# rampasek/DrVAE

Hardware: AMD Instinct MI355X
Metric: DrVAE ELBO training samples/sec (batch x L) (higher is better)
Workload: dtype f32; 1 GPU; cfg2: DrVAE bortezomib shape: 978 genes, z1=z3=100, enc-z1 800, dec-x 600, enc-z3/dec-z1 200, batch 150/GPU, L=2; global_batch=150, L=2, parallelism=dp1, launch=hipGraph replay, feed=resident, side_chain_cus=64, rccl_ranks=0, params=2321758

## Files before the change

### drvae_amd/_lib.py

```python
import ctypes as C
import os

_HERE = os.path.dirname(os.path.abspath(__file__))
LIB_PATH = os.path.join(_HERE, 'libdrvae_hip.so')

ACT = {'identity': 0, 'elu': 1, 'softplus': 2, 'sigmoid': 3, 'tanh': 4, 'relu': 5, 'leaky_relu': 6, 'selu': 7,
       'softsign': 8, 'cos': 9}
GAUSS_LOGVAR, GAUSS_SIGMA = 0, 1
REC_KIND = {'binary': 0, 'poisson': 1}
EPI_PLAIN, EPI_FWD, EPI_BWD, EPI_KLQ = 0, 1, 2, 3

_f, _i32, _i64, _u64, _p = C.c_float, C.c_int32, C.c_int64, C.c_uint64, C.c_void_p


class GemmDesc(C.Structure):
    _fields_ = [('M', _i32), ('N', _i32), ('K', _i32), ('a_kcontig', _i32), ('b_kcontig', _i32),
                ('A', _p), ('lda', _i64), ('A2', _p), ('lda2', _i64), ('K1', _i32), ('a_kscale', _p),
                ('B', _p), ('ldb', _i64), ('C', _p), ('ldc', _i64), ('alpha', _f), ('beta', _f),
                ('epilogue', _i32), ('scale', _p), ('bias', _p), ('split', _i32), ('act0', _i32), ('act1', _i32),
                ('shift0', _f), ('shift1', _f), ('resid', _p), ('ldr', _i64), ('resid_cols', _i32),
                ('yref', _p), ('ldy', _i64), ('a_colsum', _p), ('colsum_beta', _f), ('flags', _i32),
                ('pub_flag', _p), ('pub_ctr', _p), ('pub_add', _i32), ('tune', _p)]


class GemmTune(C.Structure):
    _fields_ = [('tiling', _i32), ('opt', _i32 * 10)]


class Wait(C.Structure):
    _fields_ = [('flag', _p), ('ctr', _p), ('add', _i32), ('max_spins', _i32), ('err', _p)]


class PriorKl(C.Structure):
    _fields_ = [('coef', _p), ('raw', _p), ('kl_min', _f), ('mu', _p), ('ld', _i64)]


class AdamHyper(C.Structure):
    _fields_ = [('lr', _f), ('beta1', _f), ('beta2', _f), ('eps', _f), ('weight_decay', _f), ('gscale', _f)]


class ClipRecord(C.Structure):
    _fields_ = [('norm', _f), ('coef', _f), ('skip', _i32), ('n_skipped', _i32)]


class ClipState(C.Structure):
    _fields_ = [('step', _i32), ('reserved', _i32), ('max_norm', C.c_double), ('rec', ClipRecord)]


SUMSQ_PER_BLOCK, SUMSQ_MAX_BLOCKS = 8192, 1024


class Publish(C.Structure):
    _fields_ = [('flag', _p), ('ctr', _p), ('add', _i32)]
# ... 226 lines not shown
```

### drvae_amd/csrc/optim.hip

```cpp
#include "dv_common.h"
#include <cstring>

namespace {

struct AdamC {
    float lr_over_bc1, inv_unused, bc2_sqrt, eps, wd, one_minus_b1, b2, one_minus_b2, gscale;
};

__device__ __forceinline__ void adam_consts(float lr, float b1, float b2, const int32_t* step_dev, float* step_size,
                                            float* bc2_sqrt, int n_skipped = 0) {
    const double t = (double)(step_dev[0] - n_skipped);
    const double bc1 = 1.0 - pow((double)b1, t);
    const double bc2 = 1.0 - pow((double)b2, t);
    *step_size = (float)((double)lr / bc1);
    *bc2_sqrt = (float)sqrt(bc2);
}

__device__ __forceinline__ void adam_one(float& p, float g, float& m, float& v, float step_size, float bc2_sqrt,
                                         float eps, float wd, float w1, float b2, float w2, float gscale) {
#pragma clang fp contract(off)
    g = g * gscale;
    if (wd != 0.f) g = __builtin_fmaf(wd, p, g);
    m = __builtin_fmaf(w1, g - m, m);
    v = __builtin_fmaf(w2 * g, g, v * b2);
// ... 5 lines not shown
    int bad = 0;
    for (int i = 0; i < n_halt; ++i)
        bad |= __hip_atomic_load(halt + 2 * i, __ATOMIC_RELAXED, __HIP_MEMORY_SCOPE_AGENT) != 0;
    return bad;
}

struct AdamGate {
    int32_t* flag;
    const int32_t* ctr;
    int add;
    int32_t* err;
    int max_spins;
    int64_t lo, hi;
};

template <bool CLIP>
__global__ __launch_bounds__(256) void adam_kernel(float* __restrict__ p, const float* __restrict__ g,
                                                   float* __restrict__ m, float* __restrict__ v, int64_t n, float lr,
                                                   float b1, float b2, float eps, float wd, float gscale_in,
                                                   const int32_t* __restrict__ step_dev, int vec4, AdamGate gate,
                                                   const int32_t* __restrict__ halt, int n_halt,
                                                   const dv_clip_record* __restrict__ clip) {
    __shared__ float sc[2];
    __shared__ int halted;
    bool need = false;
    if (gate.flag != nullptr) {
        const int64_t per = vec4 ? 4 : 1, span = (int64_t)blockDim.x * per;
        const int64_t bstride = (int64_t)gridDim.x * span;
        need = gate.hi > (vec4 ? ((n >> 2) << 2) : n) && gate.lo < n;
        for (int64_t e0 = blockIdx.x * span; e0 < n; e0 += bstride) need = need || (e0 < gate.hi && e0 + span > gate.lo);
    }
    if (threadIdx.x == 0) {
        int want = 0, seen = 0;
        if (need) {
            want = gate.ctr[0] + gate.add;
            seen = __hip_atomic_load(gate.flag, __ATOMIC_ACQUIRE, __HIP_MEMORY_SCOPE_AGENT);
        }
        int h = any_halt(halt, n_halt);
        if (CLIP) {
            if (clip->skip) h = 1;
            else adam_consts(lr, b1, b2, step_dev, &sc[0], &sc[1], clip->n_skipped);
        } else {
            adam_consts(lr, b1, b2, step_dev, &sc[0], &sc[1]);
        }
        if (need && seen - want < 0) {
// ... 8 lines not shown
            }
            atomicAdd(gate.err + 1, (int32_t)(wall_clock64() - t0));
            h = h || any_halt(halt, n_halt);
        }
        halted = h;
    }
    if (need) {
        __syncthreads();
        __builtin_amdgcn_fence(__ATOMIC_ACQUIRE, "agent");
    }
    __syncthreads();
    if (halted) return;
    const float step_size = sc[0], bc2_sqrt = sc[1];
    const float gscale = CLIP ? gscale_in * clip->coef : gscale_in;
    const float w1 = (float)(1.0 - (double)b1), w2 = (float)(1.0 - (double)b2);
    const int64_t stride = (int64_t)gridDim.x * blockDim.x;
    const int64_t t0 = blockIdx.x * (int64_t)blockDim.x + threadIdx.x;
    if (vec4) {
        const int64_t n4 = n >> 2;
        float4* p4 = reinterpret_cast<float4*>(p);
        const float4* g4 = reinterpret_cast<const float4*>(g);
        float4* m4 = reinterpret_cast<float4*>(m);
        float4* v4 = reinterpret_cast<float4*>(v);
        for (int64_t i = t0; i < n4; i += stride) {
            float4 pp = p4[i], gg = g4[i], mm = m4[i], vv = v4[i];
            adam_one(pp.x, gg.x, mm.x, vv.x, step_size, bc2_sqrt, eps, wd, w1, b2, w2, gscale);
            adam_one(pp.y, gg.y, mm.y, vv.y, step_size, bc2_sqrt, eps, wd, w1, b2, w2, gscale);
            adam_one(pp.z, gg.z, mm.z, vv.z, step_size, bc2_sqrt, eps, wd, w1, b2, w2, gscale);
            adam_one(pp.w, gg.w, mm.w, vv.w, step_size, bc2_sqrt, eps, wd, w1, b2, w2, gscale);
            p4[i] = pp;
            m4[i] = mm;
            v4[i] = vv;
// ... 361 lines not shown
    return c ? c + 1 : dv_src_tag;
}

extern "C" const char* dv_error_string(int code) {
    switch (code) {
        case DV_OK: return "ok";
        case DV_ERR_ARG: return "invalid argument";
        case DV_ERR_LAUNCH: return "kernel launch failed";
        case DV_ERR_UNSUPPORTED: return "unsupported configuration";
        default: return "unknown error";
    }
}

static int adam_launch(float* p, const float* g, float* m, float* v, int64_t n, float lr, float beta1, float beta2,
                       float eps, float weight_decay, float gscale, const int32_t* step_dev, const AdamGate& gate,
                       const int32_t* halt, int32_t n_halt, dv_stream_t stream, const dv_clip_record* clip = nullptr) {
    DV_REQUIRE(n >= 0 && n_halt >= 0 && (halt || n_halt == 0));
    if (n == 0) return DV_OK;
    DV_REQUIRE(p && g && m && v && step_dev);
    auto al = [](const void* q) { return (reinterpret_cast<uintptr_t>(q) & 15) == 0; };
    const int vec4 = al(p) && al(g) && al(m) && al(v);
    int64_t blocks = ((vec4 ? (n >> 2) : n) + 255) / 256;
    if (blocks < 1) blocks = 1;
    if (vec4 && gate.flag == nullptr && n >= (int64_t(16) << 20)) {
        const dim3 grid((unsigned)(blocks > 16384 ? 16384 : blocks));
        if (clip)
            hipLaunchKernelGGL(adam_stream_kernel<true>, grid, dim3(256), 0, ST(stream), p, g, m, v, n, lr, beta1, beta2, eps,
                               weight_decay, gscale, step_dev, halt, n_halt, clip);
        else
            hipLaunchKernelGGL(adam_stream_kernel<false>, grid, dim3(256), 0, ST(stream), p, g, m, v, n, lr, beta1, beta2, eps,
                               weight_decay, gscale, step_dev, halt, n_halt, clip);
        DV_RETURN_LAUNCH();
    }
    if (blocks > 2048) blocks = 2048;
    if (clip)
        hipLaunchKernelGGL(adam_kernel<true>, dim3((unsigned)blocks), dim3(256), 0, ST(stream), p, g, m, v, n, lr, beta1,
                           beta2, eps, weight_decay, gscale, step_dev, vec4, gate, halt, n_halt, clip);
    else
        hipLaunchKernelGGL(adam_kernel<false>, dim3((unsigned)blocks), dim3(256), 0, ST(stream), p, g, m, v, n, lr, beta1,
                           beta2, eps, weight_decay, gscale, step_dev, vec4, gate, halt, n_halt, clip);
    DV_RETURN_LAUNCH();
}

extern "C" int dv_adam_l2_gated(float* p, const float* g, float* m, float* v, int64_t n, const dv_adam_hyper* h,
                                const int32_t* step_dev, const dv_wait* gate, int64_t lo, int64_t hi,
                                const int32_t* halt, int32_t n_halt, dv_stream_t stream) {
    DV_REQUIRE(h != nullptr && gate != nullptr);
    DV_REQUIRE(gate->flag && gate->ctr && gate->err && gate->max_spins > 0 && lo >= 0 && hi >= lo && hi <= n);
    return adam_launch(p, g, m, v, n, h->lr, h->beta1, h->beta2, h->eps, h->weight_decay, h->gscale, step_dev,
                       AdamGate{gate->flag, gate->ctr, gate->add, gate->err, gate->max_spins, lo, hi}, halt, n_halt, stream);
}

static int adamax_launch(float* p, const float* g, float* m, float* u, int64_t n, const dv_adam_hyper* h,
                         const int32_t* step_dev, const int32_t* halt, int32_t n_halt, dv_stream_t stream,
                         const dv_clip_record* clip) {
    DV_REQUIRE(h != nullptr && n >= 0 && n_halt >= 0 && (halt || n_halt == 0));
    if (n == 0) return DV_OK;
    DV_REQUIRE(p && g && m && u && step_dev);
    int64_t blocks = (n + 255) / 256;
    if (blocks > 4096) blocks = 4096;
    if (clip)
        hipLaunchKernelGGL(adamax_kernel<true>, dim3((unsigned)blocks), dim3(256), 0, ST(stream), p, g, m, u, n, h->lr,
                           h->beta1, h->beta2, h->eps, h->weight_decay, h->gscale, step_dev, halt, n_halt, clip);
// ... 134 lines not shown
```

### drvae_amd/data.py

```python
import types

import numpy as np
import torch

from . import kernels as K


class DrVAEDataset(torch.utils.data.Dataset):

    FIELDS = ('x1', 'x2', 's', 'y', 'has_x2', 'has_y')

    def __init__(self, x1, x2, s, y, has_x2, has_y):
        n = x1.size(0)
        assert x2.size(0) == n and x1.size(1) == x2.size(1)
        assert y.size(0) == n and s.size(0) == n and has_x2.size(0) == n and has_y.size(0) == n
        self.x1, self.x2, self.s, self.y, self.has_x2, self.has_y = x1, x2, s, y, has_x2, has_y

    def __getitem__(self, index):
        return tuple(getattr(self, f)[index] for f in self.FIELDS)

    def __len__(self):
        return self.x1.size(0)

    def to(self, device):
# ... 415 lines not shown
                self._pending = self._reference_epoch()
            idx, self._pending = self._pending[0], self._pending[1:]
            return idx.to(self.ds.x1.device)
        if self.mode == 'sampler':
            return torch.multinomial(self.weights, self.global_batch, replacement=True, generator=self.gen)
        R = self.world
        parts = [m[torch.multinomial(w, c * R, replacement=True, generator=self.gen)].reshape(R, c)
                 for m, w, c in zip(self.members, self.gweights, self.group_counts) if c > 0]
        return torch.cat(parts, 1).reshape(-1)

    def feed(self, idx=None):
        if self.mode == 'sampler' and self.bucketed:
            self.engine.set_structure_universal(self.batch_size, n_tot=self._n_tot(), carry_s=self._carry)
        p = self.engine.plan
        p.feed_active = False
        idx = self.next_indices() if idx is None else idx
        if self.dp is not None and idx.numel() == self.global_batch:
            if self.mode == 'sampler':
                zero = torch.zeros((), dtype=torch.int32, device=idx.device)
                p.gcounts_dev.copy_(torch.stack([self.hx32[idx].sum() if self.engine.cfg.has_pert else zero,
                                                 self.hy32[idx].sum() if self.engine.cfg.has_y else zero]))
            idx = idx.reshape(self.world, self.batch_size)[self.rank]
        self._idx32.copy_(idx)
        K.rows_gather(p.XSRC[:p.B], self.ds.x1, self._idx32)
        if self.engine.cfg.has_pert:
            K.rows_gather(p.XSRC[p.B:], self.ds.x2, self._idx32)
        if self.engine.cfg.use_s:
            p.set_s_device(self.ds.s.reshape(-1)[idx])
        if self.mode == 'sampler':
            if self.engine.cfg.has_pert:
# ... 11 lines not shown
```

### drvae_amd/engine.py

```python
import math
import os
from collections import OrderedDict
from dataclasses import dataclass, field
from typing import List, Optional, Tuple

import numpy as np
import torch

from . import kernels as K
from . import tuning as T
from ._lib import GAUSS_LOGVAR, GAUSS_SIGMA
from .arena import N_LOSS, ParamArena, span
from .chain import X3_PARTS, _Chain, _Lin, _pad4
from .plan import LOSS_IDX, _Plan
from .schedule import DUAL, EVAL, EVALUATE, FORK_JOIN, LOSS, TRAIN, StepSchedule, StepSync, _Branch, heads_route


MATMUL_CHOICES = ('fp32',) + tuple(X3_PARTS)
assert MATMUL_CHOICES == ('fp32', 'bf16x3', 'bf16x2', 'bf16x1')


@dataclass
class StepConfig:
    kind: str = 'drvae'
# ... 294 lines not shown
            assert s is not None, 'use_s: the nuisance classes of the batch are needed'
            p = self._set_batch(x1, x2, y, has_x2, has_y, counts)
            if p.carry_s:
                sd = (s if torch.is_tensor(s) else torch.as_tensor(np.asarray(s))).reshape(-1).to(self.dev)
                if len(p.rows) != sd.numel():
                    sd = sd.index_select(0, torch.as_tensor(p.rows, device=self.dev))
                p.set_s_device(sd)
                return p
            sv = np.asarray(s.cpu() if torch.is_tensor(s) else s).astype(np.int64).reshape(-1)
            p.set_s_host(sv[p.rows])
            return p
        return self._set_batch(x1, x2, y, has_x2, has_y, counts)

    def _set_batch(self, x1, x2, y, has_x2, has_y, counts=None):
        cfg = self.cfg
        if self.universal and self.universal_ok():
            hy = np.asarray(has_y.cpu() if torch.is_tensor(has_y) else has_y).reshape(-1)
            p = self.set_structure_universal(len(hy), self.universal_pair_slots, self.universal_labeled_range,
                                             n_tot=None if counts is None else counts[0], carry_s=cfg.use_s)
            p.feed_active = False
            if counts is not None:
                p.gcounts_dev.copy_(torch.tensor([int(counts[1]), int(counts[2])], dtype=torch.int32))
            p.XSRC[:p.B].copy_(x1)
            i32 = lambda a: torch.as_tensor(np.asarray(a.cpu() if torch.is_tensor(a) else a).reshape(-1).astype(np.int32))
            if cfg.has_pert:
                if x2 is None:
                    assert has_x2 is None or not np.asarray(has_x2.cpu() if torch.is_tensor(has_x2) else has_x2).any(), \
                        'has_x2 marks pairs but x2 is None'
                    p.XSRC[p.B:].zero_()
                    p.hx_dev.zero_()
# ... 15 lines not shown
        p.XSRC[:p.B].copy_(x1.index_select(0, sel) if sel is not None else x1)
        if x2 is not None and cfg.has_pert:
            p.XSRC[p.B:].copy_(x2.index_select(0, sel) if sel is not None else x2)
        if cfg.has_y and cfg.cont:
            yv = np.asarray(y.cpu() if torch.is_tensor(y) else y).astype(np.float32).reshape(n_in, -1) \
                if y is not None else np.zeros((n_in, cfg.dim_y), np.float32)
            p.ylab.copy_(torch.from_numpy(np.ascontiguousarray(yv[rows])))
        elif cfg.has_y:
            yv = np.asarray(y.cpu() if torch.is_tensor(y) else y).astype(np.int64).reshape(-1) if y is not None \
                else np.zeros(n_in, np.int64)
            p.set_labels_host(yv[rows])
        return p

    def set_noise(self, noise):
        p, cfg = self.plan, self.cfg
        self._noise_stale = True
        t = lambda a: torch.as_tensor(np.ascontiguousarray(a), dtype=torch.float32)
        rows, L = p.rows, cfg.L
        p.EX[:p.B].copy_(t(np.asarray(noise['nx1'])[rows]))
        if p.Np:
            pr = rows[p.pair_host]
            p.EX[p.B:].copy_(t(np.asarray(noise['nx2'])[pr]))
            p.E2.copy_(t(np.asarray(noise['ez2'])[:, pr].reshape(L * p.Np, -1)))
        p.E1.copy_(t(np.asarray(noise['ez1'])[:, rows].reshape(L * p.B, -1)))
        if cfg.has_pert:
            p.E2F.copy_(t(np.asarray(noise['ez2F'])[:, rows].reshape(L * p.B, -1)))
        if cfg.has_y and p.Mf:
            ez3 = np.asarray(noise['ez3'])
            slot = p.fp_slot_host
            if p.universal:
                hy, yv, i = p.hy_dev.cpu().numpy().astype(bool), p.y_dev.cpu().numpy(), p.fp_i_host
                slot = np.where(hy[i] & (slot == yv[i]), 0, slot)
            p.E3.copy_(t(ez3[p.fp_l_host, slot, rows[p.fp_i_host]]))
        if cfg.has_y and cfg.cont:
            p.EY.copy_(t(np.asarray(noise['ey'])[:, rows].reshape(L * p.B, -1)))

    def draw_noise(self, bump=True):
        n = 1
        if self._rec == 'main' and self._tail.noise_ahead:
            self._rng_pending = n
            return
        lo = 0
        if not (self.training and self.add_noise and self.cfg.add_noise_var > 0):
            lo = self.plan.B + self.plan.Np
        self._fill_noise(self.plan, lo, keeps=self.training)
        self._noise_stale = True
        if bump:
            K.counter_add(self.rng_ctr, n)
        else:
            self._rng_pending = n

    def _fill_noise(self, p, lo=0, keeps=True):
        if p.drop_sites and keeps:
            K.fill_noise_rows(p.noise, p.noise_table[lo:], self.seed, self.rng_ctr)
            p.masks_injected = False
        else:
            K.fill_normal_rows(p.noise, p.noise_desc[lo:p.n_normal_rows], self.seed, self.rng_ctr)

    @property
    def _drop(self):
        return bool(self.training and self.plan.drop_sites)

    def dropout_sites(self):
        return [dict(s) for s in self.plan.drop_sites]

    def set_dropout_masks(self, masks):
        p = self.plan
        index = {(s['chain'], s['layer']): i for i, s in enumerate(p.drop_sites)}
        given = {(index[k] if not isinstance(k, (int, np.integer)) else int(k)): v for k, v in masks.items()}
        assert sorted(given) == list(range(len(p.drop_sites))), 'set_dropout_masks: a mask for every site'
        for i, v in given.items():
            p.drop_sites[i]['mask'].copy_(torch.as_tensor(np.ascontiguousarray(v), dtype=torch.float32))
        p.masks_injected = True
        self._noise_stale = True

    def _route(self):
        return heads_route(self, self.plan, TRAIN if self.fuse_bwd else LOSS if self.training else EVALUATE)

    def beta_pert(self):
        cfg = self.cfg
        if cfg.anneal_perturb_rate_itermax > 0:
            return anneal_coef(self.iters, cfg.anneal_perturb_rate_itermax, cfg.anneal_perturb_rate_offset)
        return 1.

    def forward(self):
        cfg, p = self.cfg, self.plan
        if not self.fuse_bwd and self.dev.type == 'cuda' and not torch.cuda.is_current_stream_capturing():
            self.join_side()
        p.set_beta(self.beta_pert())
# ... 37 lines not shown
                    z2 = None
                else:
                    K.kl_rows_fwd(*zp[0], **zp[1])
            if z2 is not None:
                K.kl_rows_fwd(*z2[0], **z2[1])
            return
        with self.branch:
            self._side_forward(Qmu, Qlv, Z1blk, r)
        if mode == FORK_JOIN:
            return
        self.branch.join()
        if self.fuse_bwd:
            return
        self._loss_scalars()

    def _encoder_forward(self, rec, r):
        cfg, p = self.cfg, self.plan
        B, Np, L, Z1 = p.B, p.Np, cfg.L, cfg.dim_z1
        sigma = cfg.add_noise_var if (self.training and self.add_noise and cfg.add_noise_var > 0) else 0.0
        Z1blk = p.ZDEC[:L * B]
        fd = p.live_feed if (self.fuse_bwd and self.training) else None
        start_park = self.sync.wait('next_step', self.step_dev, add=0) if (rec == 'main' and self._tail.tail_gated) else None
        masks = None
        if p.universal:
            gc = None
            if p.global_counts:
                gc = getattr(fd, 'gcounts', None) if fd is not None else p.gcounts_dev
                assert gc is not None, 'this plan normalises by global counts: the feed carries none (DeviceBatcher.bind(dp=...))'
            masks = dict(n_tot=p.n_tot, gcounts=gc, kl_rate=cfg.kl_qz2pz2_rate, pert_rate=cfg.pertloss_rate,
                         yl_rate=cfg.yloss_rate, beta=p.beta_dev, c_nll=p.c_nll, w_recl=p.w_recl,
                         hx=(fd.hx32 if fd is not None else p.hx_dev) if cfg.has_pert else None,
                         hy=(fd.hy32 if fd is not None else p.hy_dev) if cfg.has_y else None,
                         y=(fd.y32 if fd is not None else p.y_dev) if cfg.has_y else None,
                         c_klz2=p.c_klz2 if cfg.has_pert else None, c_yl=p.c_yl, w_pert=p.w_pert, w_yl=p.w_yl,
# ... 5 lines not shown
            lab = cfg.has_y and not cfg.cont and (not p.universal or p.one_slot is not None)
            K.batch_feed(p.XIN, fd.x1, fd.x2, fd.y32, fd.table, fd.n_batches, self.step_dev, fd.base, park=start_park,
                         pair_rows=p.pair_idx if Np else None, noise=p.EX if sigma else None, sigma=sigma,
                         has_y=p.has_y_i32 if (lab and not p.universal) else None, L=L,
                         label_r=p.label_r if (lab and not p.universal) else None,
                         fp_i=p.fp_q if lab else None, fp_lab=p.fp_lab_i32 if lab else None,
                         fp_slot=p.fp_slot_dev if lab else None, fp_cls=p.fp_cls if (lab and p.Mf) else None,
                         onehot=p.Z3IN[:, cfg.dim_z3:] if (lab and p.Mf) else None, n_classes=cfg.dim_y,
                         onehot2=p.FPIN[:, Z1:] if (lab and p.Mf) else None,
                         yf=fd.yf if (cfg.has_y and cfg.cont) else None,
                         ylab=p.ylab if (cfg.has_y and cfg.cont) else None, masks=masks)
            if cfg.use_s:
                assert p.carry_s and getattr(fd, 's32', None) is not None, 'use_s: this feed does not carry the nuisance classes'
                K.nuisance_feed(p.SOHe, p.SOHd, p.s_cls, fd.s32, table=fd.table, n_batches=fd.n_batches, ctr=self.step_dev,
                                base=fd.base, pair_rows=p.pair_idx if Np else None, L=L)
        else:
            K.rows_gather(p.XIN, p.XSRC, p.xin_idx, noise=p.EX if sigma else None, sigma=sigma, park=start_park)
        if r.sample_epi:
            Q = p.c_enc.forward(p.enc_in, heads=dict(sample=dict(
                eps=p.E12, out=p.ZDEC[:p.o3], n_src=B, seg_ptr=p.zseg_ptr, seg_rows=p.zseg_rows,
                out4=p.FPIN[:, :Z1] if r.fprop_from_heads else None, out4_ptr=p.fp_ptr_ext if r.fprop_from_heads else None)),
                drop=self._drop)
            Qmu, Qlv = Q[:, :Z1], Q[:, Z1:]
        else:
            Q = p.c_enc.forward(p.enc_in, drop=self._drop)
            Qmu, Qlv = Q[:, :Z1], Q[:, Z1:]
            K.reparam_fwd(p.ZDEC[:p.o3], Qmu, Qlv, p.E12, src_idx=p.z_src_idx)
        if cfg.has_pert:
            pub1 = self.sync.pub('z1', self.step_dev) if rec == 'main' else None
            if r.sample_epi:
                p.c_z2F.forward([Z1blk], resid=Z1blk, publish=pub1, heads=dict(sample=dict(
                    eps=p.E2F, out=p.Z2F, n_src=L * B, sub=Z1blk, out2=p.D, out3=p.ZDEC if Np else None,
# ... 435 lines not shown
        if self.clip_rec is not None:
            assert not (t and (t.adam_gated or t.cap_fork or t.side_adam)), 'a clipped sweep has no gated form'
            K.clip_norm(a.grad[:n], self.clip_state, gscale=gscale, adamax=cfg.optim_alg == 'adamax')
            step = K.adamax_l2_clip if cfg.optim_alg == 'adamax' else K.adam_l2_clip
            step(a.param[:n], a.grad[:n], a.exp_avg[:n], a.exp_avg_sq[:n], self.clip_state,
                 lr=cfg.learning_rate, weight_decay=cfg.weight_decay, gscale=gscale, halt=self.sync_err)
            return
        if t and t.adam_gated:
            if cfg.has_y:
                lc, g0 = self.L_clf[0], a.grad.storage_offset()
                lo = min(lc.dW.storage_offset(), lc.db.storage_offset()) - g0
                hi = max(lc.dW.storage_offset() + span(lc.dW), lc.db.storage_offset() + lc.db.numel()) - g0
            else:
                lo, hi = 0, 4
            kw['gate'] = self.sync.gate('clf_dw' if t.tail_gated else 'tail', self.step_dev, lo, hi)
            n = t.hs if t.side_adam else n
        if t and t.cap_fork:
            kw['gate'] = self.sync.gate('tail', self.step_dev, 0, 4)
        step(a.param[:n], a.grad[:n], a.exp_avg[:n], a.exp_avg_sq[:n], self.step_dev, lr=cfg.learning_rate,
             weight_decay=cfg.weight_decay, gscale=gscale, halt=self.sync_err, **kw)

    def clip_stats(self):
        if self.clip_rec is None:
            raise RuntimeError('clip_stats: the engine was built without max_grad_norm')
        self.join_side()
        return K.clip_record_values(self.clip_rec)

    def train_step(self, noise=None, allreduce=None):
        self.training = True
        self.join_side()
# ... 23 lines not shown
```

### drvae_amd/fit.py

```python
import time
import warnings
from collections import OrderedDict

import numpy as np
import torch

from . import engine as E
from . import metrics as MET


class EarlyStopping:

    def __init__(self, epochs, early_stop, patience=50, patience_increase=15, improvement_threshold=0.999,
                 memory_length=3, save_model_after=0):
        self.epochs, self.early_stop = epochs, early_stop
        self.patience, self.patience_increase = patience, patience_increase
        self.improvement_threshold = improvement_threshold
        self.memory_length, self.save_model_after = memory_length, save_model_after
        self.best = -np.inf
        self.rolling = np.array([], dtype=float)
        self.since_improvement = 0
        self.snapshotted = False

    def update(self, epoch, valid_obj):
# ... 736 lines not shown
            K.recon_rows(rows, ll, x, x_rec, x_std, bias=bias[:2] if bias is not None else None,
                         sd_shift=bias[2] if bias is not None else 0.0)
        else:
            K.recon_row_stats(rows, x, x_rec)
            K.nll_rows_fwd(ll, x, x_rec, x_std, mode=GAUSS_SIGMA)
        K.col_moments(None, x, x_rec, sel=sel, part=part, r_bias=bias[0] if bias is not None else None)
        K.recon_finalize(out4, rows, part, X, sel=sel, n=n, ll=ll)

    def run(self):
        m, kind = self.model, self.model.kind
        eng = m.engine()
        eng.join_side()
        eng.iters = m.finished_training_iters
        self.plan.set_beta(eng.beta_pert())
        self.graph.replay()
        eng._noise_stale = True
        if self.dp is not None:
            from . import dist as D
            D.allreduce_sum(self.pack)
            self.graph_final.replay()
        v = dict(zip(self.names, self.vec.cpu().tolist()))
        perf = OrderedDict()
        perf['losses'] = OrderedDict((k, torch.tensor(v['loss_' + k])) for k in self.loss_keys)
        parts = []
        if kind != 'pvae' and self.cont:
            for k in ('rmse', 'r2', 'pearr'):
                perf['y_' + k] = v['y_' + k]
            parts.append('Y: RMSE: {:.3f} R2: {:.3f} Pearson: {:.3f}'.format(perf['y_rmse'], perf['y_r2'], perf['y_pearr']))
        elif kind != 'pvae':
            for k in ('acc', 'auroc', 'aupr'):
                perf['y_' + k] = v['y_' + k]
# ... 16 lines not shown
```

### drvae_amd/kernels.py

```python
import ctypes as C
import math
import os
from typing import Any, NamedTuple, Optional

import torch

from . import _lib
from ._lib import ACT, EPI_BWD, EPI_FWD, EPI_KLQ, EPI_PLAIN, GAUSS_LOGVAR, GAUSS_SIGMA, GemmDesc


def _stream():
    return C.c_void_p(torch.cuda.current_stream().cuda_stream)


def _f32(t, name='tensor', any_device=False):
    if t is None:
        return None
    if not ((t.is_cuda or any_device) and t.dtype == torch.float32):
        raise RuntimeError('drvae_amd kernels need CUDA/HIP float32 tensors (%s is %s on %s); there is no CPU '
                           'fallback' % (name, t.dtype, t.device))
    if t.dim() >= 1 and t.numel() > 0 and t.stride(-1) != 1 and t.size(-1) != 1:
        raise RuntimeError('%s must have unit inner stride' % name)
    return t.data_ptr()

# ... 295 lines not shown
class Publish(NamedTuple):
    flag: Any
    ctr: Any
    add: int = 1


class Gate(NamedTuple):
    flag: Any
    ctr: Any
    add: int
    err: Any
    lo: int
    hi: int


def _wait(park):
    if park is None:
        return None
    park = Wait(*park)
    w = _lib.Wait()
    w.flag, w.ctr, w.err, w.add = _i32(park.flag), _i32(park.ctr), _i32(park.err), park.add
    w.max_spins = WAIT_SPINS if park.max_spins is None else park.max_spins
    return C.byref(w)


def _publish(pub):
    if pub is None:
        return None
    pub = Publish(*pub)
    w = _lib.Publish()
# ... 590 lines not shown
        arr[i].row_len = term[4] if len(term) > 4 else 1
    if after is None and not bump:
        _lib.check(_lib.load().dv_loss_assemble(arr, len(terms), _f32(w_elbo), _f32(w_cmpl), _f32(loss), hp, hn,
                                                _f32(accum), _stream()), 'dv_loss_assemble')
    else:
        _lib.check(_lib.load().dv_loss_assemble_after(_wait(after), arr, len(terms), _f32(w_elbo), _f32(w_cmpl), _f32(loss),
                                                      _bump(bump), hp, hn, _f32(accum), _stream()), 'dv_loss_assemble_after')


def axpby(y, x, a=1.0, b=0.0):
    assert x.is_contiguous() and y.is_contiguous() and x.numel() == y.numel()
    _lib.check(_lib.load().dv_axpby(_f32(x), a, _f32(y), b, x.numel(), _stream()), 'dv_axpby')


def adam_l2(p, g, m, v, step_dev, *, lr, beta1=0.9, beta2=0.999, eps=1e-8, weight_decay=0.0, gscale=1.0, gate=None,
            halt=None):
    assert p.is_contiguous() and g.is_contiguous() and m.is_contiguous() and v.is_contiguous()
    hp, hn = _halt(halt)
    h = _lib.AdamHyper(lr=lr, beta1=beta1, beta2=beta2, eps=eps, weight_decay=weight_decay, gscale=gscale)
    if gate is None:
        _lib.check(_lib.load().dv_adam_l2(_f32(p), _f32(g), _f32(m), _f32(v), p.numel(), C.byref(h), _i32(step_dev), hp, hn,
                                          _stream()), 'dv_adam_l2')
    else:
        gate = Gate(*gate)
        _lib.check(_lib.load().dv_adam_l2_gated(_f32(p), _f32(g), _f32(m), _f32(v), p.numel(), C.byref(h), _i32(step_dev),
                                                _wait(Wait(gate.flag, gate.ctr, gate.err, gate.add)), gate.lo, gate.hi, hp, hn,
                                                _stream()), 'dv_adam_l2_gated')


def adamax_l2(p, g, m, u, step_dev, *, lr, beta1=0.9, beta2=0.999, eps=1e-8, weight_decay=0.0, gscale=1.0, halt=None):
    assert p.is_contiguous() and g.is_contiguous() and m.is_contiguous() and u.is_contiguous()
    hp, hn = _halt(halt)
    h = _lib.AdamHyper(lr=lr, beta1=beta1, beta2=beta2, eps=eps, weight_decay=weight_decay, gscale=gscale)
    _lib.check(_lib.load().dv_adamax_l2(_f32(p), _f32(g), _f32(m), _f32(u), p.numel(), C.byref(h), _i32(step_dev), hp, hn,
                                        _stream()), 'dv_adamax_l2')


CLIP_STATE_WORDS = C.sizeof(_lib.ClipState) // 4
_CLIP_STEP, _CLIP_MAX_NORM, _CLIP_REC = (getattr(_lib.ClipState, f).offset // 4 for f in ('step', 'max_norm', 'rec'))
assert _CLIP_STEP == 0 and CLIP_STATE_WORDS % 2 == 0 and _CLIP_MAX_NORM % 2 == 0


def sumsq_partials(n):
    per, cap = _lib.SUMSQ_PER_BLOCK, _lib.SUMSQ_MAX_BLOCKS
# ... 107 lines not shown
```

### drvae_amd/schedule.py

```python
import contextlib
import ctypes
import gc
import os
import weakref
from typing import NamedTuple

import torch

from . import kernels as K
from . import tuning as T


def _masked_stream(bits, device):
    hip = ctypes.CDLL('libamdhip64.so')
    st = ctypes.c_void_p()
    arr = (ctypes.c_uint32 * len(bits))(*bits)
    with torch.cuda.device(device):
        rc = hip.hipExtStreamCreateWithCUMask(ctypes.byref(st), len(bits), arr)
    if rc != 0:
        raise RuntimeError('hipExtStreamCreateWithCUMask failed: %d' % rc)
    import atexit

    def _destroy(handle=st.value):
        try:
# ... 56 lines not shown

class Tail(NamedTuple):
    dual: bool = False
    late: bool = False
    adam_gated: bool = False
    side_adam: bool = False
    hs: int = 0
    side_loss: bool = False
    cap_fork: bool = False
    tail_gated: bool = False
    noise_ahead: bool = False
    klz2_on_main: bool = False
    fold_join: bool = False
    late_fork: bool = False
    fold_rows: bool = False


TRAIN, LOSS, EVALUATE = 'train pass', 'loss pass, separate backward', 'evaluation pass'
NLL_ROUTES = {'heads': 'NLLP', 'rec': 'NLL', 'raw_cs_eval': 'NLLC', 'raw_eval': 'NLL', 'raw_cs': 'NLLC', 'fwdbwd': 'NLL',
              'fwd': 'NLL'}


class HeadsRoute(NamedTuple):
    sample_epi: bool
    fprop_from_heads: bool
    z3_in_heads: bool
    fprop_tail: bool
    nll: str
    rows: str
    raw_last: bool
# ... 55 lines not shown
            self._forked = False
            self._ctx = torch.cuda.stream(self.side)
            self._ctx.__enter__()
        return self

    def __exit__(self, *exc):
        if self.on:
            self._ctx.__exit__(*exc)

    def join(self):
        if self.on:
            torch.cuda.current_stream().wait_stream(self.side)


_CAPTURE_STATE = ('_graphs', '_side_graph', 'noise_ahead', '_graph_key', '_graph_feed', '_graph_mmd_sig',
                  '_captured_allreduce', '_graph_noise')


class StepSchedule:

    def _init_schedule_state(self):
        self._graphs = []
        self._side_graph = None
        self.noise_ahead = False
        self._graph_key = None
        self._graph_feed = None
        self._graph_mmd_sig = None
        self._captured_allreduce = None
        self._graph_noise = None
        self._captures = {}
        self._rec = 'both'
        self._tail = Tail()
        self._after_decoder_bwd = None
        self._rng_pending = 0
        self._ctr_bumped = False
        self._noise_stale = True
        self._flag_side = None
        self._flags_ok = None
        self._side_cus = None
        self._since_poll = 0
        self._sync_host = None
        self._sync_event = None

    def stash_capture(self):
        assert self._graph_key == self.plan.key, 'stash_capture right after capture(): another plan is current'
        self._captures[self.plan.key] = {k: getattr(self, k) for k in _CAPTURE_STATE}

    def use_capture(self, key):
        cap = self._captures.get(key)
        if cap is None or cap['_graph_feed'] is not self._plans[key].live_feed or \
                cap['_graph_noise'] not in (None, self.add_noise):
            return False
        if self._graph_key != key:
            for k, v in cap.items():
                setattr(self, k, v)
            self.plan = self._plans[key]
            self._noise_stale = True
        return True

    def _mode(self):
        return EVAL if not self.fuse_bwd else DUAL if self._rec != 'both' else FORK_JOIN

    def _step_tail(self, split_kind, on_gpu=None):
        cfg, p = self.cfg, self.plan
        branch_on = self.branch.on if on_gpu is None else bool(self.concurrent and cfg.has_y and on_gpu)
        clip = cfg.max_grad_norm is not None
        if not (self.sched == 5 and self._dual_capable(on_gpu) and self._latency_bound() and
                (self._flags_usable() if on_gpu is None else on_gpu) and (cfg.has_y or not (split_kind or clip))):
            return Tail(late_fork=bool(branch_on and not self._latency_bound()))
        late_ok = bool(not cfg.cont and cfg.optim_alg == 'adam' and (self.clf_small if cfg.has_y else True))
        late = late_ok and (split_kind is True or (split_kind is False and not clip))
        side_ok, hs = self._side_adam_layout()
        side_adam = late and not split_kind and side_ok
        cap_fork = bool(split_kind == 'captured' and side_ok and late_ok and cfg.has_y and T.get('dp_fork') and not clip)
        side_loss = side_adam or (late and split_kind is True and len(self.L_decx) > 1)
        tail_gated = side_adam and (p.live_feed is not None or T.get('tail_gate') == 2)
        klz2_on_main = not cfg.cont and cfg.has_y and not p.every_row_anything
        fold_join = side_loss and cfg.has_pert and (p.B * cfg.dim_z1 + 255) // 256 <= 256 and (p.B + 3) // 4 <= 256
        noise_ahead = bool((late or cap_fork) and not p.drop_sites)
        fold_rows = bool(T.get('fold_rows') and not split_kind and not clip and not p.drop_sites and cfg.kind == 'drvae'
                         and not cfg.cont and self.clf_small and cfg.clf_z1z2 and fold_join and side_loss and noise_ahead
                         and getattr(K.z2f_post_bwd, 'fold_rows', False) and getattr(K.smalln_fwd, 'fold_rows', False))
        return Tail(dual=True, late=late, adam_gated=late and not split_kind, side_adam=side_adam, hs=hs, side_loss=side_loss,
                    cap_fork=cap_fork, tail_gated=tail_gated, noise_ahead=noise_ahead, klz2_on_main=klz2_on_main,
                    fold_join=fold_join, fold_rows=fold_rows)

    @contextlib.contextmanager
    def _recording(self, chain, tail):
        self._rec, self._tail = chain, tail
        try:
            yield
        finally:
            self._rec, self._tail = 'both', Tail()

    def _launch_sequence(self, allreduce=None, draw=True, optimizer=True):
        self.fuse_bwd = True
        try:
            if draw:
                self.draw_noise(bump=False)
            self.forward()
# ... 15 lines not shown
        self.training = True
        self.plan.set_beta(self.beta_pert())
        side = torch.cuda.Stream()
        side.wait_stream(torch.cuda.current_stream())
        with torch.cuda.stream(side):
            self.draw_noise(bump=False)
            self._rng_pending = 0
            self.forward()
            self.backward()
        torch.cuda.current_stream().wait_stream(side)
        torch.cuda.synchronize()
        self._graphs = []
        self._side_graph = None
        tail = self._step_tail(split_for_allreduce)
        self.noise_ahead = tail.noise_ahead
        self._noise_stale = True
        gc.collect()
        gc_was_on = gc.isenabled()
        gc.disable()
        try:
            with self._recording('main' if tail.dual else 'both', tail):
                self._capture_main(split_for_allreduce)
            if tail.dual:
                self.sync_side_counters()
                self.flag_side.wait_stream(torch.cuda.current_stream())
                gs = torch.cuda.CUDAGraph()
                with torch.cuda.graph(gs, stream=self.flag_side), self._recording('side', tail):
                    self._launch_sequence(draw=False, optimizer=False)
                self._side_graph = gs
        finally:
            if gc_was_on:
# ... 82 lines not shown
                for _ in range(4):
                    self.replay()
                e0, e1 = torch.cuda.Event(enable_timing=True), torch.cuda.Event(enable_timing=True)
                e0.record()
                for _ in range(steps):
                    self.replay()
                e1.record()
                e1.synchronize()
                t = e0.elapsed_time(e1)
            if t < best[1]:
                best = (n, t)
        torch.cuda.synchronize()
        for dst, src in zip(state, keep):
            dst.copy_(src)
        self.iters = iters
        self._noise_stale = True
        self.plan.set_beta(self.beta_pert())
        torch.cuda.synchronize()
        self._side_cus = best[0]
        return best[0]

    @property
    def flag_side(self):
        if self._flag_side is None:
            self._flag_side = torch.cuda.Stream(device=self.dev)
        return self._flag_side

    def _probe(self, side):
        probe = torch.zeros(4, dtype=torch.int32, device=self.dev)
        torch.cuda.synchronize()
        K.flag_wait(probe[0:1], probe[1:2], probe[2:4], add=1, max_spins=20000)
# ... 83 lines not shown
            g = torch.cuda.CUDAGraph()
            with torch.cuda.graph(g):
                self._launch_sequence(allreduce=self._captured_allreduce)
            self._graphs = [g]

    def replay(self, allreduce=None):
        assert self._graph_key == self.plan.key, 'batch structure changed: capture again'
        assert self._graph_feed is self.plan.live_feed, 'input source changed (epoch feed <-> explicit batch): capture again'
        assert self._graph_mmd_sig == getattr(self.plan, 'mmd_sig', None), \
            'use_MMD: the nuisance classes of the batch changed (the penalty compares row sets): capture again'
        self.plan.set_beta(self.beta_pert())
        self.plan.masks_injected = False
        if self.noise_ahead and self._noise_stale:
            self._fill_noise(self.plan)
            self._noise_stale = False
        self._graphs[0].replay()
        if self._side_graph is not None:
            with torch.cuda.stream(self.flag_side):
                self._side_graph.replay()
        if len(self._graphs) == 3:
            a = self.arena
            w_early = allreduce.start(a.xchg[a.late_end:])
            self._graphs[1].replay()
            w_late = allreduce.start(a.xchg[:a.late_end])
            allreduce.finish(w_early)
            allreduce.finish(w_late)
            self._graphs[2].replay()
        elif len(self._graphs) == 2:
            if self._side_graph is not None:
                torch.cuda.current_stream().wait_stream(self.flag_side)
# ... 7 lines not shown
```

### drvae_amd/tuning.py

```python
import os

DEFAULTS = {
    'sched': 5,
    'fuse_heads': 1,
    'raw_heads': 1,
    'tail_gate': 1,
    'concurrent': 1,
    'nll_cs': 1,
    'mmd_explicit': 1,
    'fold_rows': 1,
    'dp_fork': 1,
}

CHOICES = {'sched': (3, 5), 'fuse_heads': (0, 1), 'raw_heads': (1, 2), 'tail_gate': (1, 2), 'concurrent': (0, 1),
           'nll_cs': (1, 2), 'mmd_explicit': (0, 1), 'dp_fork': (0, 1), 'fold_rows': (0, 1)}


def _parse():
    out = dict(DEFAULTS)
    for kv in filter(None, os.environ.get('DRVAE_TUNE', '').split(',')):
        k, _, v = kv.partition('=')
        k = k.strip()
        if k not in DEFAULTS:
            raise ValueError('DRVAE_TUNE: unknown switch %r (known: %s)' % (k, ', '.join(sorted(DEFAULTS))))
        out[k] = int(v)
        if out[k] not in CHOICES[k]:
            raise ValueError('DRVAE_TUNE: %s=%d is not a schedule (known: %s)' % (k, out[k], CHOICES[k]))
    return out


# ... 14 lines not shown
```

### include/drvae_hip.h

```cpp
#ifndef DRVAE_HIP_H
#define DRVAE_HIP_H

#include <stdint.h>

#ifdef __cplusplus
extern "C" {
#endif

typedef void* dv_stream_t;

#define DV_ABI_VERSION 12

enum { DV_OK = 0, DV_ERR_ARG = -1, DV_ERR_LAUNCH = -2, DV_ERR_UNSUPPORTED = -3 };

enum {
    DV_ACT_IDENTITY = 0, DV_ACT_ELU = 1, DV_ACT_SOFTPLUS = 2, DV_ACT_SIGMOID = 3, DV_ACT_TANH = 4,
    DV_ACT_RELU = 5, DV_ACT_LEAKY_RELU = 6, DV_ACT_SELU = 7, DV_ACT_SOFTSIGN = 8, DV_ACT_COS = 9
};

enum { DV_GAUSS_LOGVAR = 0, DV_GAUSS_SIGMA = 1 };

enum { DV_EPI_PLAIN = 0, DV_EPI_FWD = 1, DV_EPI_BWD = 2, DV_EPI_KLQ = 3 };

int dv_abi_version(void);
// ... 563 lines not shown
int dv_axpby(const float* x, float a, float* y, float b, int64_t n, dv_stream_t stream);

typedef struct dv_adam_hyper {
    float lr;
    float beta1;
    float beta2;
    float eps;
    float weight_decay;
    float gscale;
} dv_adam_hyper;
int dv_adam_l2(float* p, const float* g, float* m, float* v, int64_t n, const dv_adam_hyper* h,
               const int32_t* step_dev, const int32_t* halt, int32_t n_halt, dv_stream_t stream);
int dv_adam_l2_gated(float* p, const float* g, float* m, float* v, int64_t n, const dv_adam_hyper* h,
                     const int32_t* step_dev, const dv_wait* gate, int64_t lo, int64_t hi, const int32_t* halt,
                     int32_t n_halt, dv_stream_t stream);
int dv_adamax_l2(float* p, const float* g, float* m, float* u, int64_t n, const dv_adam_hyper* h,
                 const int32_t* step_dev, const int32_t* halt, int32_t n_halt, dv_stream_t stream);
typedef struct dv_clip_record {
    float norm;
    float coef;
    int32_t skip;
    int32_t n_skipped;
} dv_clip_record;
typedef struct dv_clip_state {
    int32_t step;
    int32_t reserved;
    double max_norm;
    dv_clip_record rec;
} dv_clip_state;
#define DV_SUMSQ_PER_BLOCK 8192
// ... 18 lines not shown
```

Baseline: 1.659 million samples/s.

## Gather next step's encoder inputs inside the gated Adam kernel as a rider

```diff
diff --git a/drvae_amd/_lib.py b/drvae_amd/_lib.py
--- a/drvae_amd/_lib.py
+++ b/drvae_amd/_lib.py
@@ -37,6 +37,11 @@
 
 class AdamHyper(C.Structure):
     _fields_ = [('lr', _f), ('beta1', _f), ('beta2', _f), ('eps', _f), ('weight_decay', _f), ('gscale', _f)]
+
+
+class AdamRider(C.Structure):
+    _fields_ = [('halt', _p), ('n_halt', _i32), ('n', _i32), ('W', _i32), ('sigma', _f), ('src', _p), ('lds', _i64),
+                ('idx', _p), ('noise', _p), ('ldn', _i64), ('out', _p), ('ldo', _i64)]
 
 
 class ClipRecord(C.Structure):
diff --git a/drvae_amd/csrc/optim.hip b/drvae_amd/csrc/optim.hip
--- a/drvae_amd/csrc/optim.hip
+++ b/drvae_amd/csrc/optim.hip
@@ -43,21 +43,86 @@
     int64_t lo, hi;
 };
 
-template <bool CLIP>
+struct AdamRider {
+    const float* src;
+    int64_t lds;
+    const int32_t* idx;
+    const float* noise;
+    int64_t ldn;
+    float* out;
+    int64_t ldo;
+    int n, W;
+    float sigma;
+    unsigned nblk;
+};
+
+__device__ __forceinline__ void adam_rider_block(const AdamRider& rd, const AdamGate& gate, const int32_t* __restrict__ halt,
+                                                 int n_halt, int* halted) {
+    const int lane = threadIdx.x & 63;
+    const int wave = blockIdx.x * (blockDim.x >> 6) + (threadIdx.x >> 6), nwave = (int)rd.nblk * (blockDim.x >> 6);
+    int64_t row0 = wave;
+    if (rd.idx != nullptr && wave < rd.n) row0 = rd.idx[wave];
+    if (threadIdx.x == 0) {
+        int h = any_halt(halt, n_halt);
+        const int want = gate.ctr[0] + gate.add;
+        int k = 0;
+        while (__hip_atomic_load(gate.flag, __ATOMIC_ACQUIRE, __HIP_MEMORY_SCOPE_AGENT) - want < 0) {
+            __builtin_amdgcn_s_sleep(4);
+            if (++k > gate.max_spins) {
+                atomicExch(gate.err, 1);
+                h = 1;
+                break;
+            }
+        }
+        *halted = h || any_halt(halt, n_halt);
+    }
+    __syncthreads();
+    __builtin_amdgcn_fence(__ATOMIC_ACQUIRE, "agent");
+    if (*halted) return;
+    constexpr int U = 8;
+    for (int r = wave; r < rd.n; r += nwave) {
+        const int64_t sr = r == wave ? row0 : (rd.idx ? (int64_t)rd.idx[r] : (int64_t)r);
+        const float* __restrict__ s = rd.src + sr * rd.lds;
+        const float* __restrict__ z = rd.noise ? rd.noise + (int64_t)r * rd.ldn : nullptr;
+        float* __restrict__ o = rd.out + (int64_t)r * rd.ldo;
+        for (int d0 = lane; d0 < rd.W; d0 += 64 * U) {
+            float x[U], e[U];
+#pragma unroll
+            for (int u = 0; u < U; ++u) {
+                const int d = d0 + 64 * u;
+                x[u] = d < rd.W ? s[d] : 0.f;
+                e[u] = (z && d < rd.W) ? z[d] : 0.f;
+            }
+#pragma unroll
+            for (int u = 0; u < U; ++u) {
+                const int d = d0 + 64 * u;
+                if (d < rd.W) o[d] = z ? __builtin_fmaf(rd.sigma, e[u], x[u]) : x[u];
+            }
+        }
+    }
+}
+
+template <bool CLIP, bool RIDER>
 __global__ __launch_bounds__(256) void adam_kernel(float* __restrict__ p, const float* __restrict__ g,
                                                    float* __restrict__ m, float* __restrict__ v, int64_t n, float lr,
                                                    float b1, float b2, float eps, float wd, float gscale_in,
                                                    const int32_t* __restrict__ step_dev, int vec4, AdamGate gate,
                                                    const int32_t* __restrict__ halt, int n_halt,
-                                                   const dv_clip_record* __restrict__ clip) {
+                                                   const dv_clip_record* __restrict__ clip, AdamRider rd) {
     __shared__ float sc[2];
     __shared__ int halted;
+    if (RIDER && blockIdx.x < rd.nblk) {
+        adam_rider_block(rd, gate, halt, n_halt, &halted);
+        return;
+    }
+    const unsigned nrd = RIDER ? rd.nblk : 0u;
+    const unsigned bid = blockIdx.x - nrd, nblocks = gridDim.x - nrd;
     bool need = false;
     if (gate.flag != nullptr) {
         const int64_t per = vec4 ? 4 : 1, span = (int64_t)blockDim.x * per;
-        const int64_t bstride = (int64_t)gridDim.x * span;
+        const int64_t bstride = (int64_t)nblocks * span;
         need = gate.hi > (vec4 ? ((n >> 2) << 2) : n) && gate.lo < n;
-        for (int64_t e0 = blockIdx.x * span; e0 < n; e0 += bstride) need = need || (e0 < gate.hi && e0 + span > gate.lo);
+        for (int64_t e0 = bid * span; e0 < n; e0 += bstride) need = need || (e0 < gate.hi && e0 + span > gate.lo);
     }
     if (threadIdx.x == 0) {
         int want = 0, seen = 0;
@@ -96,8 +161,8 @@
     const float step_size = sc[0], bc2_sqrt = sc[1];
     const float gscale = CLIP ? gscale_in * clip->coef : gscale_in;
     const float w1 = (float)(1.0 - (double)b1), w2 = (float)(1.0 - (double)b2);
-    const int64_t stride = (int64_t)gridDim.x * blockDim.x;
-    const int64_t t0 = blockIdx.x * (int64_t)blockDim.x + threadIdx.x;
+    const int64_t stride = (int64_t)nblocks * blockDim.x;
+    const int64_t t0 = bid * (int64_t)blockDim.x + threadIdx.x;
     if (vec4) {
         const int64_t n4 = n >> 2;
         float4* p4 = reinterpret_cast<float4*>(p);
@@ -489,7 +554,8 @@
 
 static int adam_launch(float* p, const float* g, float* m, float* v, int64_t n, float lr, float beta1, float beta2,
                        float eps, float weight_decay, float gscale, const int32_t* step_dev, const AdamGate& gate,
-                       const int32_t* halt, int32_t n_halt, dv_stream_t stream, const dv_clip_record* clip = nullptr) {
+                       const int32_t* halt, int32_t n_halt, dv_stream_t stream, const dv_clip_record* clip = nullptr,
+                       const AdamRider* rider = nullptr) {
     DV_REQUIRE(n >= 0 && n_halt >= 0 && (halt || n_halt == 0));
     if (n == 0) return DV_OK;
     DV_REQUIRE(p && g && m && v && step_dev);
@@ -508,12 +574,15 @@
         DV_RETURN_LAUNCH();
     }
     if (blocks > 2048) blocks = 2048;
-    if (clip)
-        hipLaunchKernelGGL(adam_kernel<true>, dim3((unsigned)blocks), dim3(256), 0, ST(stream), p, g, m, v, n, lr, beta1,
-                           beta2, eps, weight_decay, gscale, step_dev, vec4, gate, halt, n_halt, clip);
+    if (rider)
+        hipLaunchKernelGGL((adam_kernel<false, true>), dim3((unsigned)blocks + rider->nblk), dim3(256), 0, ST(stream), p, g, m, v,
+                           n, lr, beta1, beta2, eps, weight_decay, gscale, step_dev, vec4, gate, halt, n_halt, clip, *rider);
+    else if (clip)
+        hipLaunchKernelGGL((adam_kernel<true, false>), dim3((unsigned)blocks), dim3(256), 0, ST(stream), p, g, m, v, n, lr, beta1,
+                           beta2, eps, weight_decay, gscale, step_dev, vec4, gate, halt, n_halt, clip, AdamRider{});
     else
-        hipLaunchKernelGGL(adam_kernel<false>, dim3((unsigned)blocks), dim3(256), 0, ST(stream), p, g, m, v, n, lr, beta1,
-                           beta2, eps, weight_decay, gscale, step_dev, vec4, gate, halt, n_halt, clip);
+        hipLaunchKernelGGL((adam_kernel<false, false>), dim3((unsigned)blocks), dim3(256), 0, ST(stream), p, g, m, v, n, lr, beta1,
+                           beta2, eps, weight_decay, gscale, step_dev, vec4, gate, halt, n_halt, clip, AdamRider{});
     DV_RETURN_LAUNCH();
 }
 
@@ -522,6 +591,22 @@
                                 const int32_t* halt, int32_t n_halt, dv_stream_t stream) {
     DV_REQUIRE(h != nullptr && gate != nullptr);
     DV_REQUIRE(gate->flag && gate->ctr && gate->err && gate->max_spins > 0 && lo >= 0 && hi >= lo && hi <= n);
+    if (n_halt < 0) {
+        DV_REQUIRE(n_halt == -1 && halt != nullptr);
+        const dv_adam_rider* r = reinterpret_cast<const dv_adam_rider*>(halt);
+        DV_REQUIRE(r->n >= 0 && r->W >= 0 && r->n_halt >= 0 && (r->halt || r->n_halt == 0) && n > 0);
+        const int64_t total = (int64_t)r->n * r->W;
+        if (total == 0)
+            return adam_launch(p, g, m, v, n, h->lr, h->beta1, h->beta2, h->eps, h->weight_decay, h->gscale, step_dev,
+                               AdamGate{gate->flag, gate->ctr, gate->add, gate->err, gate->max_spins, lo, hi}, r->halt,
+                               r->n_halt, stream);
+        DV_REQUIRE(r->src && r->out);
+        const unsigned nblk = (unsigned)(r->n > 4 * DV_ADAM_RIDER_MAX_BLOCKS ? DV_ADAM_RIDER_MAX_BLOCKS : (r->n + 3) / 4);
+        const AdamRider rd{r->src, r->lds, r->idx, r->noise, r->ldn, r->out, r->ldo, r->n, r->W, r->sigma, nblk};
+        return adam_launch(p, g, m, v, n, h->lr, h->beta1, h->beta2, h->eps, h->weight_decay, h->gscale, step_dev,
+                           AdamGate{gate->flag, gate->ctr, gate->add, gate->err, gate->max_spins, lo, hi}, r->halt, r->n_halt,
+                           stream, nullptr, &rd);
+    }
     return adam_launch(p, g, m, v, n, h->lr, h->beta1, h->beta2, h->eps, h->weight_decay, h->gscale, step_dev,
                        AdamGate{gate->flag, gate->ctr, gate->add, gate->err, gate->max_spins, lo, hi}, halt, n_halt, stream);
 }
diff --git a/drvae_amd/data.py b/drvae_amd/data.py
--- a/drvae_amd/data.py
+++ b/drvae_amd/data.py
@@ -453,6 +453,7 @@
             self.engine.set_structure_universal(self.batch_size, n_tot=self._n_tot(), carry_s=self._carry)
         p = self.engine.plan
         p.feed_active = False
+        self.engine.inputs_stale(host_feed=True)
         idx = self.next_indices() if idx is None else idx
         if self.dp is not None and idx.numel() == self.global_batch:
             if self.mode == 'sampler':
diff --git a/drvae_amd/engine.py b/drvae_amd/engine.py
--- a/drvae_amd/engine.py
+++ b/drvae_amd/engine.py
@@ -332,6 +332,7 @@
 
     def _set_batch(self, x1, x2, y, has_x2, has_y, counts=None):
         cfg = self.cfg
+        self.inputs_stale(host_feed=False)
         if self.universal and self.universal_ok():
             hy = np.asarray(has_y.cpu() if torch.is_tensor(has_y) else has_y).reshape(-1)
             p = self.set_structure_universal(len(hy), self.universal_pair_slots, self.universal_labeled_range,
@@ -377,7 +378,7 @@
 
     def set_noise(self, noise):
         p, cfg = self.plan, self.cfg
-        self._noise_stale = True
+        self.inputs_stale()
         t = lambda a: torch.as_tensor(np.ascontiguousarray(a), dtype=torch.float32)
         rows, L = p.rows, cfg.L
         p.EX[:p.B].copy_(t(np.asarray(noise['nx1'])[rows]))
@@ -407,7 +408,7 @@
         if not (self.training and self.add_noise and self.cfg.add_noise_var > 0):
             lo = self.plan.B + self.plan.Np
         self._fill_noise(self.plan, lo, keeps=self.training)
-        self._noise_stale = True
+        self.inputs_stale()
         if bump:
             K.counter_add(self.rng_ctr, n)
         else:
@@ -435,7 +436,7 @@
         for i, v in given.items():
             p.drop_sites[i]['mask'].copy_(torch.as_tensor(np.ascontiguousarray(v), dtype=torch.float32))
         p.masks_injected = True
-        self._noise_stale = True
+        self.inputs_stale()
 
     def _route(self):
         return heads_route(self, self.plan, TRAIN if self.fuse_bwd else LOSS if self.training else EVALUATE)
@@ -503,10 +504,18 @@
             return
         self._loss_scalars()
 
+    def _input_sigma(self):
+        cfg = self.cfg
+        return cfg.add_noise_var if (self.training and self.add_noise and cfg.add_noise_var > 0) else 0.0
+
+    def _gather_inputs(self, p, sigma, park=None):
+        K.rows_gather(p.XIN, p.XSRC, p.xin_idx, noise=p.EX if sigma else None, sigma=sigma, park=park)
+        self._xin_stale = True
+
     def _encoder_forward(self, rec, r):
         cfg, p = self.cfg, self.plan
         B, Np, L, Z1 = p.B, p.Np, cfg.L, cfg.dim_z1
-        sigma = cfg.add_noise_var if (self.training and self.add_noise and cfg.add_noise_var > 0) else 0.0
+        sigma = self._input_sigma()
         Z1blk = p.ZDEC[:L * B]
         fd = p.live_feed if (self.fuse_bwd and self.training) else None
         start_park = self.sync.wait('next_step', self.step_dev, add=0) if (rec == 'main' and self._tail.tail_gated) else None
@@ -542,8 +551,8 @@
                 assert p.carry_s and getattr(fd, 's32', None) is not None, 'use_s: this feed does not carry the nuisance classes'
                 K.nuisance_feed(p.SOHe, p.SOHd, p.s_cls, fd.s32, table=fd.table, n_batches=fd.n_batches, ctr=self.step_dev,
                                 base=fd.base, pair_rows=p.pair_idx if Np else None, L=L)
-        else:
-            K.rows_gather(p.XIN, p.XSRC, p.xin_idx, noise=p.EX if sigma else None, sigma=sigma, park=start_park)
+        elif not (rec == 'main' and self._tail.xin_ahead):
+            self._gather_inputs(p, sigma, park=start_park)
         if r.sample_epi:
             Q = p.c_enc.forward(p.enc_in, heads=dict(sample=dict(
                 eps=p.E12, out=p.ZDEC[:p.o3], n_src=B, seg_ptr=p.zseg_ptr, seg_rows=p.zseg_rows,
@@ -1009,6 +1018,9 @@
             else:
                 lo, hi = 0, 4
             kw['gate'] = self.sync.gate('clf_dw' if t.tail_gated else 'tail', self.step_dev, lo, hi)
+            if t.xin_ahead:
+                p, sigma = self.plan, self._input_sigma()
+                kw['rider'] = K.XinRider(p.XIN, p.XSRC, p.xin_idx, p.EX if sigma else None, sigma)
             n = t.hs if t.side_adam else n
         if t and t.cap_fork:
             kw['gate'] = self.sync.gate('tail', self.step_dev, 0, 4)
diff --git a/drvae_amd/fit.py b/drvae_amd/fit.py
--- a/drvae_amd/fit.py
+++ b/drvae_amd/fit.py
@@ -774,7 +774,7 @@
         eng.iters = m.finished_training_iters
         self.plan.set_beta(eng.beta_pert())
         self.graph.replay()
-        eng._noise_stale = True
+        eng.inputs_stale()
         if self.dp is not None:
             from . import dist as D
             D.allreduce_sum(self.pack)
diff --git a/drvae_amd/kernels.py b/drvae_amd/kernels.py
--- a/drvae_amd/kernels.py
+++ b/drvae_amd/kernels.py
@@ -333,6 +333,14 @@
     hi: int
 
 
+class XinRider(NamedTuple):
+    out: Any
+    src: Any
+    idx: Any = None
+    noise: Any = None
+    sigma: float = 0.0
+
+
 def _wait(park):
     if park is None:
         return None
@@ -953,10 +961,22 @@
 
 
 def adam_l2(p, g, m, v, step_dev, *, lr, beta1=0.9, beta2=0.999, eps=1e-8, weight_decay=0.0, gscale=1.0, gate=None,
-            halt=None):
+            halt=None, rider=None):
     assert p.is_contiguous() and g.is_contiguous() and m.is_contiguous() and v.is_contiguous()
     hp, hn = _halt(halt)
     h = _lib.AdamHyper(lr=lr, beta1=beta1, beta2=beta2, eps=eps, weight_decay=weight_decay, gscale=gscale)
+    if rider is not None:
+        assert gate is not None, 'the rider parks on the sweep\'s gate'
+        rider, gate = XinRider(*rider), Gate(*gate)
+        rd = _lib.AdamRider(halt=hp, n_halt=hn, n=rider.out.shape[0], W=rider.src.shape[1], sigma=rider.sigma,
+                            src=_f32(rider.src), lds=_ld(rider.src), idx=_i32(rider.idx), noise=_f32(rider.noise),
+                            ldn=_ld(rider.noise), out=_f32(rider.out), ldo=_ld(rider.out))
+        assert rider.out.shape[1] >= rd.W and (rider.idx is None or rider.idx.numel() >= rd.n) and \
+            (rider.noise is None or (rider.noise.shape[0] >= rd.n and rider.noise.shape[1] >= rd.W))
+        _lib.check(_lib.load().dv_adam_l2_gated(_f32(p), _f32(g), _f32(m), _f32(v), p.numel(), C.byref(h), _i32(step_dev),
+                                                _wait(Wait(gate.flag, gate.ctr, gate.err, gate.add)), gate.lo, gate.hi,
+                                                C.addressof(rd), -1, _stream()), 'dv_adam_l2_gated (rider)')
+        return
     if gate is None:
         _lib.check(_lib.load().dv_adam_l2(_f32(p), _f32(g), _f32(m), _f32(v), p.numel(), C.byref(h), _i32(step_dev), hp, hn,
                                           _stream()), 'dv_adam_l2')
@@ -967,6 +987,9 @@
                                                 _stream()), 'dv_adam_l2_gated')
 
 
+adam_l2.xin_rider = True
+
+
 def adamax_l2(p, g, m, u, step_dev, *, lr, beta1=0.9, beta2=0.999, eps=1e-8, weight_decay=0.0, gscale=1.0, halt=None):
     assert p.is_contiguous() and g.is_contiguous() and m.is_contiguous() and u.is_contiguous()
     hp, hn = _halt(halt)
diff --git a/drvae_amd/schedule.py b/drvae_amd/schedule.py
--- a/drvae_amd/schedule.py
+++ b/drvae_amd/schedule.py
@@ -94,6 +94,7 @@
     fold_join: bool = False
     late_fork: bool = False
     fold_rows: bool = False
+    xin_ahead: bool = False
 
 
 TRAIN, LOSS, EVALUATE = 'train pass', 'loss pass, separate backward', 'evaluation pass'
@@ -179,7 +180,7 @@
 
 
 _CAPTURE_STATE = ('_graphs', '_side_graph', 'noise_ahead', '_graph_key', '_graph_feed', '_graph_mmd_sig',
-                  '_captured_allreduce', '_graph_noise')
+                  '_captured_allreduce', '_graph_noise', 'xin_ahead', '_xin_sigma')
 
 
 class StepSchedule:
@@ -193,6 +194,8 @@
         self._graph_mmd_sig = None
         self._captured_allreduce = None
         self._graph_noise = None
+        self.xin_ahead = False
+        self._xin_sigma = 0.0
         self._captures = {}
         self._rec = 'both'
         self._tail = Tail()
@@ -200,6 +203,8 @@
         self._rng_pending = 0
         self._ctr_bumped = False
         self._noise_stale = True
+        self._xin_stale = True
+        self._host_feed = False
         self._flag_side = None
         self._flags_ok = None
         self._side_cus = None
@@ -220,8 +225,14 @@
             for k, v in cap.items():
                 setattr(self, k, v)
             self.plan = self._plans[key]
-            self._noise_stale = True
+            self.inputs_stale()
         return True
+
+    def inputs_stale(self, host_feed=None):
+        self._noise_stale = True
+        self._xin_stale = True
+        if host_feed is not None:
+            self._host_feed = bool(host_feed)
 
     def _mode(self):
         return EVAL if not self.fuse_bwd else DUAL if self._rec != 'both' else FORK_JOIN
@@ -246,9 +257,12 @@
         fold_rows = bool(T.get('fold_rows') and not split_kind and not clip and not p.drop_sites and cfg.kind == 'drvae'
                          and not cfg.cont and self.clf_small and cfg.clf_z1z2 and fold_join and side_loss and noise_ahead
                          and getattr(K.z2f_post_bwd, 'fold_rows', False) and getattr(K.smalln_fwd, 'fold_rows', False))
-        return Tail(dual=True, late=late, adam_gated=late and not split_kind, side_adam=side_adam, hs=hs, side_loss=side_loss,
+        adam_gated = late and not split_kind
+        xin_ahead = bool(T.get('xin_ahead') and adam_gated and not tail_gated and noise_ahead and not clip and not p.drop_sites
+                         and p.live_feed is None and not self._host_feed and getattr(K.adam_l2, 'xin_rider', False))
+        return Tail(dual=True, late=late, adam_gated=adam_gated, side_adam=side_adam, hs=hs, side_loss=side_loss,
                     cap_fork=cap_fork, tail_gated=tail_gated, noise_ahead=noise_ahead, klz2_on_main=klz2_on_main,
-                    fold_join=fold_join, fold_rows=fold_rows)
+                    fold_join=fold_join, fold_rows=fold_rows, xin_ahead=xin_ahead)
 
     @contextlib.contextmanager
     def _recording(self, chain, tail):
@@ -294,7 +308,8 @@
         self._side_graph = None
         tail = self._step_tail(split_for_allreduce)
         self.noise_ahead = tail.noise_ahead
-        self._noise_stale = True
+        self.xin_ahead, self._xin_sigma = tail.xin_ahead, self._input_sigma()
+        self.inputs_stale()
         gc.collect()
         gc_was_on = gc.isenabled()
         gc.disable()
@@ -407,7 +422,7 @@
         for dst, src in zip(state, keep):
             dst.copy_(src)
         self.iters = iters
-        self._noise_stale = True
+        self.inputs_stale()
         self.plan.set_beta(self.beta_pert())
         torch.cuda.synchronize()
         self._side_cus = best[0]
@@ -521,6 +536,10 @@
         if self.noise_ahead and self._noise_stale:
             self._fill_noise(self.plan)
             self._noise_stale = False
+        if self.xin_ahead:
+            if self._xin_stale:
+                self._gather_inputs(self.plan, self._xin_sigma)
+            self._xin_stale = False
         self._graphs[0].replay()
         if self._side_graph is not None:
             with torch.cuda.stream(self.flag_side):
diff --git a/drvae_amd/tuning.py b/drvae_amd/tuning.py
--- a/drvae_amd/tuning.py
+++ b/drvae_amd/tuning.py
@@ -9,11 +9,12 @@
     'nll_cs': 1,
     'mmd_explicit': 1,
     'fold_rows': 1,
+    'xin_ahead': 1,
     'dp_fork': 1,
 }
 
 CHOICES = {'sched': (3, 5), 'fuse_heads': (0, 1), 'raw_heads': (1, 2), 'tail_gate': (1, 2), 'concurrent': (0, 1),
-           'nll_cs': (1, 2), 'mmd_explicit': (0, 1), 'dp_fork': (0, 1), 'fold_rows': (0, 1)}
+           'nll_cs': (1, 2), 'mmd_explicit': (0, 1), 'dp_fork': (0, 1), 'fold_rows': (0, 1), 'xin_ahead': (0, 1)}
 
 
 def _parse():
diff --git a/include/drvae_hip.h b/include/drvae_hip.h
--- a/include/drvae_hip.h
+++ b/include/drvae_hip.h
@@ -601,6 +601,21 @@
 int dv_adam_l2_gated(float* p, const float* g, float* m, float* v, int64_t n, const dv_adam_hyper* h,
                      const int32_t* step_dev, const dv_wait* gate, int64_t lo, int64_t hi, const int32_t* halt,
                      int32_t n_halt, dv_stream_t stream);
+typedef struct dv_adam_rider {
+    const int32_t* halt;
+    int32_t n_halt;
+    int32_t n;
+    int32_t W;
+    float sigma;
+    const float* src;
+    int64_t lds;
+    const int32_t* idx;
+    const float* noise;
+    int64_t ldn;
+    float* out;
+    int64_t ldo;
+} dv_adam_rider;
+#define DV_ADAM_RIDER_MAX_BLOCKS 64
 int dv_adamax_l2(float* p, const float* g, float* m, float* u, int64_t n, const dv_adam_hyper* h,
                  const int32_t* step_dev, const int32_t* halt, int32_t n_halt, dv_stream_t stream);
 typedef struct dv_clip_record {
```

Measured after the change: 1.674 million samples/s (median of 6 runs). Within noise of the previous version (+0.9%).
